# YyzHarry/imbalanced-regression

Hardware: NVIDIA H100
Metric: images/sec (higher is better)
Workload: dtype bf16

## Files before the change

imbalanced-regression_b200/csrc/conv_igemm.cu:

```cuda
#include <stdlib.h>
#include "common.cuh"
#include "tc.cuh"
#include "conv.cuh"

namespace dirb200 {
using namespace tc;

constexpr int BM = 128;
constexpr int BK = 64;
constexpr int kProducerThreads = 128;
constexpr int kThreads = 384;
constexpr int kMaxTaps = 25;
constexpr int kMaxSmemBytes = 232448;

struct IgemmParams {
  const __nv_bfloat16* src;
  int n, hs, ws, cs;
  int hm, wm;
  int kh, kw, stride, pad;
  int transposed;
  int cls_on, cls_py, cls_px, full_h, full_w;
  int ntaps_c;
  int tap_list[kMaxTaps];
  long long tap_eoff[kMaxTaps];
  unsigned short tap_r[kMaxTaps], tap_s[kMaxTaps];
  FastDiv fd_hw, fd_wm, fd_cpb, fd_kw, fd_ntiles, fd_persplit;
  int cpb;
  long long pixels;
  int num_kblocks;
  int kblocks_per_split;
  int total_chunks;
  int m_tiles, n_tiles;
  int num_tiles;
  int a_mode;
  int i2c_stride, i2c_lo;
  int ldc;
  void* out;
  float* stat_out;
  const float* epi_scale;
  const float* epi_shift;
  const __nv_bfloat16* epi_res;
  int epi_relu;
  const __nv_bfloat16* bst_y;
  const float* bst_scale;
  const float* bst_shift;
};

template <int BN, bool STAGED_EPI>
struct Cfg {
  static constexpr int kABytes = BM * BK * 2;
  static constexpr int kBBytes = BN * BK * 2;
  static constexpr int kStageBytes = kABytes + kBBytes;
  static constexpr int kStages = BN == 128 ? (STAGED_EPI ? 5 : 6) : 8;
  static constexpr int kBarOffset = kStages * kStageBytes;
  static constexpr int kStageRowBytes = BN * 2 + 16;
  static constexpr int kEpiWarpBytes = 16 * kStageRowBytes;
  static constexpr int kEpiOffset = kBarOffset + 256;
  static constexpr int kStatWarpBytes = 2 * BN * 4;
  static constexpr int kStatOffset = kEpiOffset + (STAGED_EPI ? 8 * kEpiWarpBytes : 0);
  static constexpr int kSmemBytes = kStatOffset + (STAGED_EPI ? 8 * kStatWarpBytes : 0) + 1024;
  static_assert(kSmemBytes <= kMaxSmemBytes, "shared memory budget");
};

__device__ __forceinline__ uint32_t pack_pixel(long long p, const IgemmParams& P) {
  if (p >= P.pixels) return 0u;
  uint32_t n, rem, y, x;
  P.fd_hw.divmod(static_cast<uint32_t>(p), n, rem);
  P.fd_wm.divmod(rem, y, x);
  return 0x80000000u | (n << 18) | (y << 9) | x;
}

struct RowPre {
  int nb, yb, xb;
};
__device__ __forceinline__ RowPre row_pre(const IgemmParams& P, uint32_t pk) {
  RowPre rp;
  const int n = (pk >> 18) & 0x1FFF;
  int y = (pk >> 9) & 0x1FF, x = pk & 0x1FF;
  if (P.cls_on) {
    y = 2 * y + P.cls_py;
    x = 2 * x + P.cls_px;
  }
  rp.nb = n * P.hs;
  if (!P.transposed) {
    rp.yb = y * P.stride - P.pad;
    rp.xb = x * P.stride - P.pad;
  } else {
    rp.yb = y + P.pad;
    rp.xb = x + P.pad;
  }
  if (!(pk >> 31)) rp.yb = -(1 << 28);
  return rp;
}

__device__ __forceinline__ const __nv_bfloat16* tap_source(const IgemmParams& P, const RowPre& rp, int r, int s,
                                                           int coff, bool& ok) {
  int hi, wi;
  ok = true;
  if (!P.transposed) {
    hi = rp.yb + r;
    wi = rp.xb + s;
  } else {
    hi = rp.yb - r;
    wi = rp.xb - s;
    if (P.stride == 2) {
      ok = ((hi | wi) & 1) == 0;
      hi >>= 1;
      wi >>= 1;
    }
  }
  ok = ok && static_cast<unsigned>(hi) < static_cast<unsigned>(P.hs) &&
       static_cast<unsigned>(wi) < static_cast<unsigned>(P.ws);
  return ok ? P.src + (static_cast<size_t>(rp.nb + hi) * P.ws + wi) * P.cs + coff : P.src;
}
template <int BN, bool WGRAD, bool STEM, bool ATMA = false, bool AFFINE = false, bool BSTAT = false>
__global__ void __launch_bounds__(kThreads, 1)
igemm_kernel(const __grid_constant__ CUtensorMap tmap_b, const __grid_constant__ CUtensorMap tmap_a,
             const IgemmParams P) {
  using C = Cfg<BN, !WGRAD>;
  static_assert(BN == 64 || BN == 128, "tile width: one m64n64 / m64n128 wgmma per warpgroup and k step");
  static_assert(!ATMA || !STEM, "TMA-fed A operand: not for the stem");
  static_assert(!AFFINE || (!WGRAD && !STEM), "folded-BN epilogue: non-stem fprop GEMMs only");
  static_assert(!BSTAT || (ATMA && !WGRAD && !AFFINE), "BN-backward moments in the epilogue: TMA-fed dgrad GEMMs only");
  extern __shared__ uint8_t smem_raw[];
  const uint32_t smem_base = (smem_u32(smem_raw) + 1023u) & ~1023u;
  uint8_t* const smem_gen = smem_raw + (smem_base - smem_u32(smem_raw));
  const uint32_t bar_base = smem_base + C::kBarOffset;
  auto a_addr = [&](int s) { return smem_base + s * C::kStageBytes; };
  auto b_addr = [&](int s) { return smem_base + s * C::kStageBytes + C::kABytes; };
  constexpr uint32_t nstages = C::kStages;
  auto full_bar = [&](int s) { return bar_base + 8u * s; };
  auto empty_bar = [&](int s) { return bar_base + 8u * (C::kStages + s); };
  const int warp = static_cast<int>(threadIdx.x >> 5), lane = threadIdx.x & 31;

  int tile_first, tile_end, tile_step, fixed_n = 0;
  if constexpr (WGRAD) {
    tile_first = blockIdx.x; tile_end = P.num_tiles; tile_step = gridDim.x;
  } else {
    uint32_t gi, nn;
    P.fd_ntiles.divmod(blockIdx.x, gi, nn);
    fixed_n = static_cast<int>(nn);
    tile_first = static_cast<int>(gi);
    tile_end = P.m_tiles;
    tile_step = static_cast<int>(P.fd_ntiles.div(gridDim.x - 1u - nn)) + 1;
  }
  auto decode_tile = [&](int t, int& split, int& m_tile, int& n_tile, int& kb_begin, int& nk) {
    if constexpr (WGRAD) {
      uint32_t sp, rem, mt, nt;
      P.fd_persplit.divmod(static_cast<uint32_t>(t), sp, rem);
      P.fd_ntiles.divmod(rem, mt, nt);
      split = static_cast<int>(sp);
      m_tile = static_cast<int>(mt);
      n_tile = static_cast<int>(nt);
      kb_begin = split * P.kblocks_per_split;
      const int kb_end = min(P.num_kblocks, kb_begin + P.kblocks_per_split);
      nk = max(0, kb_end - kb_begin);
    } else {
      split = 0;
      m_tile = t;
      n_tile = fixed_n;
      kb_begin = 0;
      nk = P.num_kblocks;
    }
  };

  if (threadIdx.x == 0) {
    for (int s = 0; s < C::kStages; ++s) {
      mbar_init(full_bar(s), ATMA ? 1 : kProducerThreads + 1);
      mbar_init(empty_bar(s), 8);
    }
    fence_barrier_init();
  }
  __syncthreads();

  if (warp < 4) {
    if constexpr (!ATMA) {
      const int j = lane & 7;
      const int q = lane >> 3;
      uint32_t rs = 0, rph = 0;
      for (int t = tile_first; t < tile_end; t += tile_step) {
        int split, m_tile, n_tile, kb_begin, nk;
        decode_tile(t, split, m_tile, n_tile, kb_begin, nk);
        const int n0 = n_tile * BN;
        long long off8[8];
        uint32_t mask8[8];
        int chunk_r = 0, chunk_s = 0, chunk_c0 = 0;
        bool chunk_ok = true;
        uint32_t tile_off = 0;
        if constexpr (!WGRAD) {
          const RowPre rp = row_pre(P, pack_pixel(static_cast<long long>(m_tile) * BM + warp * 32 + lane, P));
          const bool rvalid = rp.yb > -(1 << 27);
          int oy = rp.yb, ox = rp.xb;
          if (P.transposed && P.stride == 2) { oy >>= 1; ox >>= 1; }
          const long long my_off = (static_cast<long long>(rp.nb + oy) * P.ws + ox) * P.cs;
          uint32_t vy = 0, vx = 0;
          if (rvalid) {
            const int nky = P.kh, nkx = STEM ? 4 : P.kw;
            for (int r = 0; r < nky; ++r) {
              int h = P.transposed ? rp.yb - r : rp.yb + r;
              bool ok = true;
              if (P.transposed && P.stride == 2) { ok = (h & 1) == 0; h >>= 1; }
              vy |= (ok && static_cast<unsigned>(h) < static_cast<unsigned>(P.hs) ? 1u : 0u) << r;
            }
            for (int c = 0; c < nkx; ++c) {
              int w = P.transposed ? rp.xb - c : rp.xb + c;
              bool ok = true;
              if (P.transposed && P.stride == 2) { ok = (w & 1) == 0; w >>= 1; }
              vx |= (ok && static_cast<unsigned>(w) < static_cast<unsigned>(P.ws) ? 1u : 0u) << c;
            }
          }
          uint32_t my_mask;
          if constexpr (STEM) {
            my_mask = vy | (vx << 8);
          } else {
            my_mask = 0;
            for (int r = 0; r < P.kh; ++r)
              if ((vy >> r) & 1u) my_mask |= vx << (r * P.kw);
          }
#pragma unroll
          for (int i = 0; i < 8; ++i) {
            const int row = 4 * i + q;
            const long long o = __shfl_sync(0xffffffffu, my_off, row);
            const uint32_t m = __shfl_sync(0xffffffffu, my_mask, row);
            if constexpr (STEM) {
              off8[i] = o + (j >> 1) * P.cs + (j & 1) * 8;
              mask8[i] = ((m >> (8 + (j >> 1))) & 1u) ? (m & 0xFu) : 0u;
            } else {
              off8[i] = o + j * 8;
              mask8[i] = m;
            }
          }
          tile_off = warp * 32 * 128;
        } else {
          const int chunk = warp >> 1;
          const int gchunk = m_tile * 2 + chunk;
          chunk_ok = gchunk < P.total_chunks;
          if constexpr (STEM) {
            chunk_r = gchunk;
          } else {
            uint32_t tap, cb, cr, csx;
            P.fd_cpb.divmod(static_cast<uint32_t>(gchunk), tap, cb);
            P.fd_kw.divmod(tap, cr, csx);
            chunk_c0 = static_cast<int>(cb) * 64;
            chunk_r = static_cast<int>(cr);
            chunk_s = static_cast<int>(csx);
          }
          tile_off = chunk * 8192 + (warp & 1) * 32 * 128;
        }
        int tc = 0, cb = 0;
        long long stem_toff = 0;
        for (int it = 0; it < nk; ++it) {
          const int s = static_cast<int>(rs);
          mbar_wait(empty_bar(s), rph ^ 1u);
          if (++rs == nstages) { rs = 0; rph ^= 1u; }
          const int kb = kb_begin + it;
          const uint32_t dst_base = a_addr(s) + tile_off;
          int kcoord = kb;
          if constexpr (!WGRAD) {
            int tp;
            long long toff;
            if constexpr (STEM) {
              tp = kb;
              toff = stem_toff;
              stem_toff += static_cast<long long>(P.ws) * P.cs;
            } else {
              tp = P.tap_list[tc];
              toff = P.tap_eoff[tc] + cb * 64;
              kcoord = tp * P.cpb + cb;
              if (++cb == P.cpb) { cb = 0; ++tc; }
            }
#pragma unroll
            for (int i = 0; i < 8; ++i) {
              const int row = 4 * i + q;
              const bool ok = (mask8[i] >> tp) & 1u;
              const __nv_bfloat16* src = ok ? P.src + (off8[i] + toff) : P.src;
              cp_async16(dst_base + row * 128 + ((j ^ (row & 7)) << 4), src, ok ? 16u : 0u);
            }
          } else {
            const uint32_t mypk = chunk_ok ? pack_pixel(static_cast<long long>(kb) * 64 + (warp & 1) * 32 + lane, P) : 0u;
            const RowPre rp = row_pre(P, mypk);
            bool myok;
            const __nv_bfloat16* myptr = tap_source(P, rp, chunk_r, STEM ? 0 : chunk_s, STEM ? 0 : chunk_c0, myok);
            const unsigned long long myaddr = reinterpret_cast<unsigned long long>(myptr);
            uint32_t okbits;
            if constexpr (STEM) {
              okbits = 0;
              const bool rowok = (mypk >> 31) && static_cast<unsigned>(rp.yb + chunk_r) < static_cast<unsigned>(P.hs);
              for (int sp = 0; sp < 4; ++sp)
                okbits |= (rowok && static_cast<unsigned>(rp.xb + sp) < static_cast<unsigned>(P.ws) ? 1u : 0u) << sp;
            } else {
              okbits = myok ? 1u : 0u;
            }
            unsigned long long rowaddr = myaddr;
            if constexpr (STEM)
              rowaddr = reinterpret_cast<unsigned long long>(
                  P.src + ((static_cast<long long>(rp.nb + rp.yb + chunk_r) * P.ws + rp.xb) * P.cs));
#pragma unroll
            for (int i = 0; i < 8; ++i) {
              const int row = 4 * i + q;
              const unsigned long long a = __shfl_sync(0xffffffffu, rowaddr, row);
              const uint32_t okb = __shfl_sync(0xffffffffu, okbits, row);
              const bool ok = STEM ? ((okb >> (j >> 1)) & 1u) : (okb & 1u);
              const __nv_bfloat16* src = reinterpret_cast<const __nv_bfloat16*>(a) + j * 8;
              cp_async16(dst_base + row * 128 + ((j ^ (row & 7)) << 4), ok ? src : P.src, ok ? 16u : 0u);
            }
          }
          if (warp == 0) {
            if (elect_one()) {
              mbar_arrive_expect_tx(full_bar(s), C::kBBytes);
              if constexpr (!WGRAD) {
                tma_load_2d(b_addr(s), &tmap_b, full_bar(s), kcoord * BK, n0);
              } else {
#pragma unroll
                for (int i = 0; i < BN / 64; ++i)
                  tma_load_2d(b_addr(s) + i * 8192, &tmap_b, full_bar(s), n0 + 64 * i, kb * 64);
              }
            }
            __syncwarp();
          }
          cp_async_mbar_arrive_noinc(full_bar(s));
        }
      }
    } else if (warp == 0) {
      uint32_t rs = 0, rph = 0;
      for (int t = tile_first; t < tile_end; t += tile_step) {
        int split, m_tile, n_tile, kb_begin, nk;
        decode_tile(t, split, m_tile, n_tile, kb_begin, nk);
        const int n0 = n_tile * BN;
        int tile_w0 = 0, tile_h0 = 0, tile_n0 = 0;
        if constexpr (!WGRAD) {
          if (P.a_mode == 2) {
            uint32_t tn, rem, y0, x0;
            P.fd_hw.divmod(static_cast<uint32_t>(m_tile) * BM, tn, rem);
            P.fd_wm.divmod(rem, y0, x0);
            tile_n0 = static_cast<int>(tn);
            tile_w0 = static_cast<int>(x0) * P.i2c_stride + P.i2c_lo;
            tile_h0 = static_cast<int>(y0) * P.i2c_stride + P.i2c_lo;
          }
        }
        int tc = 0, cb = 0;
        for (int it = 0; it < nk; ++it) {
          const int s = static_cast<int>(rs);
          mbar_wait(empty_bar(s), rph ^ 1u);
          if (++rs == nstages) { rs = 0; rph ^= 1u; }
          const int kb = kb_begin + it;
          if (elect_one()) {
            if constexpr (!WGRAD) {
              mbar_arrive_expect_tx(full_bar(s), C::kBBytes + C::kABytes);
              if (P.a_mode == 1)
                tma_load_2d(a_addr(s), &tmap_a, full_bar(s), kb * BK, m_tile * BM);
              else
                tma_load_im2col_4d(a_addr(s), &tmap_a, full_bar(s), cb * BK, tile_w0, tile_h0, tile_n0,
                                   P.tap_s[tc], P.tap_r[tc]);
              tma_load_2d(b_addr(s), &tmap_b, full_bar(s), (P.tap_list[tc] * P.cpb + cb) * BK, n0);
            } else {
              const int nchunks = min(2, P.total_chunks - 2 * m_tile);
              mbar_arrive_expect_tx(full_bar(s), C::kBBytes + nchunks * 8192);
              if (P.a_mode == 1) {
                for (int i = 0; i < nchunks; ++i)
                  tma_load_2d(a_addr(s) + i * 8192, &tmap_a, full_bar(s), (2 * m_tile + i) * 64, kb * 64);
              } else {
                uint32_t n0i, rem, y0, x0;
                P.fd_hw.divmod(static_cast<uint32_t>(kb) * 64u, n0i, rem);
                P.fd_wm.divmod(rem, y0, x0);
                for (int i = 0; i < nchunks; ++i) {
                  uint32_t tap, cbk, r, sx;
                  P.fd_cpb.divmod(static_cast<uint32_t>(2 * m_tile + i), tap, cbk);
                  P.fd_kw.divmod(tap, r, sx);
                  tma_load_im2col_4d(a_addr(s) + i * 8192, &tmap_a, full_bar(s), static_cast<int>(cbk) * 64,
                                     static_cast<int>(x0) * P.i2c_stride + P.i2c_lo,
                                     static_cast<int>(y0) * P.i2c_stride + P.i2c_lo, static_cast<int>(n0i),
                                     static_cast<uint16_t>(sx), static_cast<uint16_t>(r));
                }
              }
#pragma unroll
              for (int i = 0; i < BN / 64; ++i)
                tma_load_2d(b_addr(s) + i * 8192, &tmap_b, full_bar(s), n0 + 64 * i, kb * 64);
            }
          }
          if constexpr (!WGRAD) {
            if (++cb == P.cpb) { cb = 0; ++tc; }
          }
          __syncwarp();
        }
      }
    }
    return;
  }

  const int g = (warp >> 2) - 1;
  const int wq = warp & 3;
  const int ew = g * 4 + wq;
  const int fr = lane >> 2, fc = 2 * (lane & 3);
  float* const stat_sm = reinterpret_cast<float*>(smem_gen + C::kStatOffset) + ew * (2 * BN);
  if constexpr (!WGRAD) {
    if (P.stat_out != nullptr)
      for (int i = lane; i < 2 * BN; i += 32) stat_sm[i] = 0.f;
  }
  constexpr uint32_t kLbo = WGRAD ? 8192u : 16u;
  constexpr uint32_t kadv = WGRAD ? (2048u >> 4) : (32u >> 4);
  constexpr int kT = WGRAD ? 1 : 0;
  float acc[BN / 2];
  uint32_t rs = 0, rph = 0;
  for (int t = tile_first; t < tile_end; t += tile_step) {
    int split, m_tile, n_tile, kb_begin, nk;
    decode_tile(t, split, m_tile, n_tile, kb_begin, nk);
    int prev = 0;
    for (int it = 0; it < nk; ++it) {
      const int s = static_cast<int>(rs);
      mbar_wait(full_bar(s), rph);
      if (++rs == nstages) { rs = 0; rph ^= 1u; }
      if constexpr (!ATMA) fence_proxy_async();
      const uint64_t adesc = make_smem_desc(a_addr(s) + g * 8192, kLbo, 1024u);
      const uint64_t bdesc = make_smem_desc(b_addr(s), kLbo, 1024u);
      wgmma_fence_operands(acc);
      wgmma_fence();
#pragma unroll
      for (int k = 0; k < BK / 16; ++k)
        wgmma_bf16<BN, kT, kT>(acc, adesc + static_cast<uint64_t>(k * kadv), bdesc + static_cast<uint64_t>(k * kadv),
                               (it > 0 || k > 0) ? 1u : 0u);
      wgmma_commit();
      wgmma_fence_operands(acc);
      if (it > 0) {
        wgmma_wait<1>();
        if (lane == 0) mbar_arrive(empty_bar(prev));
      }
      prev = s;
    }
    wgmma_wait<0>();
    wgmma_fence_operands(acc);
    if (nk > 0 && lane == 0) mbar_arrive(empty_bar(prev));
    const int n0 = n_tile * BN;

    if constexpr (!WGRAD) {
      const uint32_t stage_base = smem_base + C::kEpiOffset + ew * C::kEpiWarpBytes;
      const bool relu_now = AFFINE && P.epi_relu && P.epi_res == nullptr;
#pragma unroll
      for (int j = 0; j < BN / 8; ++j) {
        const int col = 8 * j + fc;
        float v0 = acc[4 * j], v1 = acc[4 * j + 1], v2 = acc[4 * j + 2], v3 = acc[4 * j + 3];
        if constexpr (AFFINE) {
          const float2 a = __ldg(reinterpret_cast<const float2*>(P.epi_scale + n0 + col));
          const float2 b = __ldg(reinterpret_cast<const float2*>(P.epi_shift + n0 + col));
          v0 = fmaf(v0, a.x, b.x); v1 = fmaf(v1, a.y, b.y); v2 = fmaf(v2, a.x, b.x); v3 = fmaf(v3, a.y, b.y);
          if (relu_now) { v0 = fmaxf(v0, 0.f); v1 = fmaxf(v1, 0.f); v2 = fmaxf(v2, 0.f); v3 = fmaxf(v3, 0.f); }
        }
        __nv_bfloat162 h0 = __floats2bfloat162_rn(v0, v1), h1 = __floats2bfloat162_rn(v2, v3);
        asm volatile("st.shared.b32 [%0], %1;" ::"r"(stage_base + fr * C::kStageRowBytes + col * 2),
                     "r"(*reinterpret_cast<uint32_t*>(&h0)) : "memory");
        asm volatile("st.shared.b32 [%0], %1;" ::"r"(stage_base + (fr + 8) * C::kStageRowBytes + col * 2),
                     "r"(*reinterpret_cast<uint32_t*>(&h1)) : "memory");
      }
      __syncwarp();
      constexpr int kLanesPerRow = BN * 2 / 16;
      constexpr int kRowsPerIter = 32 / kLanesPerRow;
      constexpr int kIters = 16 / kRowsPerIter;
      const int sub = lane / kLanesPerRow, col16 = lane % kLanesPerRow;
      const long long p0 = static_cast<long long>(m_tile) * BM + g * 64 + wq * 16;
      __nv_bfloat16* out_cols = reinterpret_cast<__nv_bfloat16*>(P.out) + n0 + col16 * 8;
#pragma unroll
      for (int i = 0; i < kIters; ++i) {
        const int rl = i * kRowsPerIter + sub;
        const long long p = p0 + rl;
        int orow = (p < P.pixels && nk > 0) ? static_cast<int>(p) : -1;
        if (orow >= 0 && P.cls_on) {
          const uint32_t pk = pack_pixel(p, P);
          const int n = (pk >> 18) & 0x1FFF, yy = (pk >> 9) & 0x1FF, xx = pk & 0x1FF;
          orow = (n * P.full_h + 2 * yy + P.cls_py) * P.full_w + 2 * xx + P.cls_px;
        }
        if (orow >= 0) {
          uint4 val;
          asm volatile("ld.shared.v4.b32 {%0, %1, %2, %3}, [%4];"
                       : "=r"(val.x), "=r"(val.y), "=r"(val.z), "=r"(val.w)
                       : "r"(stage_base + rl * C::kStageRowBytes + col16 * 16));
          if constexpr (AFFINE) {
            if (P.epi_res != nullptr) {
              const uint4 rv = *reinterpret_cast<const uint4*>(P.epi_res + n0 + col16 * 8 + static_cast<long long>(orow) * P.ldc);
              uint32_t o[4] = {val.x, val.y, val.z, val.w};
              const uint32_t rr[4] = {rv.x, rv.y, rv.z, rv.w};
#pragma unroll
              for (int e = 0; e < 4; ++e) {
                float lo = __uint_as_float(o[e] << 16) + __uint_as_float(rr[e] << 16);
                float hi = __uint_as_float(o[e] & 0xffff0000u) + __uint_as_float(rr[e] & 0xffff0000u);
                if (P.epi_relu) { lo = fmaxf(lo, 0.f); hi = fmaxf(hi, 0.f); }
                __nv_bfloat162 h = __floats2bfloat162_rn(lo, hi);
                o[e] = *reinterpret_cast<uint32_t*>(&h);
              }
              val = make_uint4(o[0], o[1], o[2], o[3]);
            }
          }
          *reinterpret_cast<uint4*>(out_cols + static_cast<long long>(orow) * P.ldc) = val;
        }
      }
      if (BSTAT || P.stat_out != nullptr) {
#pragma unroll
        for (int h = 0; h < BN / 64; ++h) {
          const int col = 2 * (lane + 32 * h);
          float s0 = 0.f, s1 = 0.f, q0 = 0.f, q1 = 0.f;
          float2 bsc = make_float2(0.f, 0.f), bsh = bsc;
          if constexpr (BSTAT) {
            bsc = __ldg(reinterpret_cast<const float2*>(P.bst_scale + n0 + col));
            bsh = __ldg(reinterpret_cast<const float2*>(P.bst_shift + n0 + col));
          }
#pragma unroll
          for (int r = 0; r < 16; ++r) {
            uint32_t w;
            asm volatile("ld.shared.b32 %0, [%1];" : "=r"(w) : "r"(stage_base + r * C::kStageRowBytes + col * 2));
            float g0 = __uint_as_float(w << 16), g1 = __uint_as_float(w & 0xffff0000u);
            if constexpr (BSTAT) {
              const long long p = p0 + r;
              const uint32_t yw = p < P.pixels ? __ldg(reinterpret_cast<const unsigned int*>(P.bst_y + p * P.ldc + n0 + col)) : 0u;
              const float y0 = __uint_as_float(yw << 16), y1 = __uint_as_float(yw & 0xffff0000u);
              if (!(fmaf(y0, bsc.x, bsh.x) > 0.f)) g0 = 0.f;
              if (!(fmaf(y1, bsc.y, bsh.y) > 0.f)) g1 = 0.f;
              s0 += g0; s1 += g1;
              q0 = fmaf(g0, y0, q0); q1 = fmaf(g1, y1, q1);
            } else {
              s0 += g0; s1 += g1;
              q0 = fmaf(g0, g0, q0); q1 = fmaf(g1, g1, q1);
            }
          }
          stat_sm[col] += s0;
          stat_sm[col + 1] += s1;
          stat_sm[BN + col] += q0;
          stat_sm[BN + col + 1] += q1;
        }
      }
      __syncwarp();
    } else {
      const int ktot = P.total_chunks * 64;
      const int krow = m_tile * BM + g * 64 + wq * 16 + fr;
      float* out = reinterpret_cast<float*>(P.out) + (static_cast<size_t>(split) * P.ldc + n0) * ktot;
#pragma unroll
      for (int j = 0; j < BN / 8; ++j) {
        const size_t c0 = static_cast<size_t>(8 * j + fc) * ktot;
#pragma unroll
        for (int e = 0; e < 2; ++e) {
          if (krow < ktot) out[c0 + e * ktot + krow] = nk > 0 ? acc[4 * j + e] : 0.f;
          if (krow + 8 < ktot) out[c0 + e * ktot + krow + 8] = nk > 0 ? acc[4 * j + 2 + e] : 0.f;
        }
      }
    }
  }
  if constexpr (!WGRAD) {
    if (P.stat_out != nullptr) {
      asm volatile("bar.sync 1, 256;" ::: "memory");
      const float* all = reinterpret_cast<const float*>(smem_gen + C::kStatOffset);
      float* dst = P.stat_out + static_cast<size_t>(blockIdx.x) * 2 * P.ldc + fixed_n * BN;
      for (int o = static_cast<int>(threadIdx.x) - kProducerThreads; o < 2 * BN; o += kThreads - kProducerThreads) {
        const int k = o / BN, col = o - k * BN;
        const float v = ((all[o] + all[2 * BN + o]) + (all[4 * BN + o] + all[6 * BN + o])) +
                        ((all[8 * BN + o] + all[10 * BN + o]) + (all[12 * BN + o] + all[14 * BN + o]));
        dst[static_cast<size_t>(k) * P.ldc + col] = v;
      }
    }
  }
}

typedef CUresult (*EncodeTiledFn)(CUtensorMap*, CUtensorMapDataType, cuuint32_t, void*, const cuuint64_t*,
                                  const cuuint64_t*, const cuuint32_t*, const cuuint32_t*, CUtensorMapInterleave,
                                  CUtensorMapSwizzle, CUtensorMapL2promotion, CUtensorMapFloatOOBfill);

static EncodeTiledFn encode_fn() {
  static EncodeTiledFn fn = nullptr;
  if (!fn) {
    void* p = nullptr;
    cudaDriverEntryPointQueryResult q;
    if (cudaGetDriverEntryPoint("cuTensorMapEncodeTiled", &p, cudaEnableDefault, &q) == cudaSuccess &&
        q == cudaDriverEntryPointSuccess)
      fn = reinterpret_cast<EncodeTiledFn>(p);
  }
  return fn;
}

int make_tmap_bf16_2d(CUtensorMap* tm, const void* ptr, uint64_t inner, uint64_t outer, uint64_t row_stride_bytes,
                      uint32_t box_outer) {
  EncodeTiledFn fn = encode_fn();
  if (!fn) {
    set_error("cuTensorMapEncodeTiled entry point not available");
    return DIRB200_ERR_CUDA;
  }
  cuuint64_t dims[2] = {inner, outer};
  cuuint64_t strides[1] = {row_stride_bytes};
  cuuint32_t box[2] = {64, box_outer};
  cuuint32_t estr[2] = {1, 1};
  CUresult r = fn(tm, CU_TENSOR_MAP_DATA_TYPE_BFLOAT16, 2, const_cast<void*>(ptr), dims, strides, box, estr,
                  CU_TENSOR_MAP_INTERLEAVE_NONE, CU_TENSOR_MAP_SWIZZLE_128B, CU_TENSOR_MAP_L2_PROMOTION_L2_256B,
                  CU_TENSOR_MAP_FLOAT_OOB_FILL_NONE);
  if (r != CUDA_SUCCESS) {
    set_error("cuTensorMapEncodeTiled failed (%d) inner=%llu outer=%llu stride=%llu", (int)r,
              (unsigned long long)inner, (unsigned long long)outer, (unsigned long long)row_stride_bytes);
    return DIRB200_ERR_CUDA;
  }
  return DIRB200_OK;
}

typedef CUresult (*EncodeIm2colFn)(CUtensorMap*, CUtensorMapDataType, cuuint32_t, void*, const cuuint64_t*,
                                   const cuuint64_t*, const int*, const int*, cuuint32_t, cuuint32_t, const cuuint32_t*,
                                   CUtensorMapInterleave, CUtensorMapSwizzle, CUtensorMapL2promotion,
                                   CUtensorMapFloatOOBfill);
int make_tmap_im2col_bf16(CUtensorMap* tm, const void* ptr, int c, int w, int h, int n, int lower_w, int lower_h,
                          int upper_w, int upper_h, int trav, int pixels_per_col) {
  static EncodeIm2colFn fn = nullptr;
  if (!fn) {
    void* p = nullptr;
    cudaDriverEntryPointQueryResult q;
    if (cudaGetDriverEntryPoint("cuTensorMapEncodeIm2col", &p, cudaEnableDefault, &q) == cudaSuccess &&
        q == cudaDriverEntryPointSuccess)
      fn = reinterpret_cast<EncodeIm2colFn>(p);
  }
  if (!fn) {
    set_error("cuTensorMapEncodeIm2col entry point not available");
    return DIRB200_ERR_CUDA;
  }
  cuuint64_t dims[4] = {(cuuint64_t)c, (cuuint64_t)w, (cuuint64_t)h, (cuuint64_t)n};
  cuuint64_t strides[3] = {(cuuint64_t)c * 2, (cuuint64_t)w * c * 2, (cuuint64_t)h * w * c * 2};
  int lower[2] = {lower_w, lower_h}, upper[2] = {upper_w, upper_h};
  cuuint32_t estr[4] = {1, (cuuint32_t)trav, (cuuint32_t)trav, 1};
  CUresult r = fn(tm, CU_TENSOR_MAP_DATA_TYPE_BFLOAT16, 4, const_cast<void*>(ptr), dims, strides, lower, upper, 64,
                  (cuuint32_t)pixels_per_col, estr, CU_TENSOR_MAP_INTERLEAVE_NONE, CU_TENSOR_MAP_SWIZZLE_128B,
                  CU_TENSOR_MAP_L2_PROMOTION_L2_256B, CU_TENSOR_MAP_FLOAT_OOB_FILL_NONE);
  if (r != CUDA_SUCCESS) {
    set_error("cuTensorMapEncodeIm2col failed (%d) c=%d w=%d h=%d n=%d lower=%d,%d upper=%d,%d stride=%d", (int)r, c, w, h,
              n, lower_w, lower_h, upper_w, upper_h, trav);
    return DIRB200_ERR_CUDA;
  }
  int drv = 0;
  if (cudaDriverGetVersion(&drv) == cudaSuccess && drv <= 13010 && (size_t)c * w * h * n * 2 < 131072)
    reinterpret_cast<uint64_t*>(tm)[1] &= ~(1ull << 21);
  return DIRB200_OK;
}
static thread_local StatLayout t_last_layout{};

static IgemmParams finish_params(const IgemmParams& P) {
  IgemmParams Q = P;
  Q.fd_hw = make_fastdiv(static_cast<uint32_t>(Q.hm * Q.wm));
  Q.fd_wm = make_fastdiv(static_cast<uint32_t>(Q.wm));
  Q.fd_cpb = make_fastdiv(static_cast<uint32_t>(Q.cpb > 0 ? Q.cpb : 1));
  Q.fd_kw = make_fastdiv(static_cast<uint32_t>(Q.kw > 0 ? Q.kw : 1));
  Q.fd_ntiles = make_fastdiv(static_cast<uint32_t>(Q.n_tiles > 0 ? Q.n_tiles : 1));
  Q.fd_persplit = make_fastdiv(static_cast<uint32_t>(Q.m_tiles * Q.n_tiles > 0 ? Q.m_tiles * Q.n_tiles : 1));
  const int nt = Q.ntaps_c < kMaxTaps ? Q.ntaps_c : kMaxTaps;
  for (int i = 0; i < kMaxTaps; ++i) {
    Q.tap_eoff[i] = 0;
    Q.tap_r[i] = Q.tap_s[i] = 0;
  }
  for (int i = 0; i < nt && Q.kw > 0; ++i) {
    const int tp = Q.tap_list[i];
    int r = tp / Q.kw, sx = tp - r * Q.kw;
    if (Q.transposed && Q.cls_on) {
      Q.tap_r[i] = static_cast<unsigned short>((Q.cls_py + Q.pad - r) / 2 - Q.i2c_lo);
      Q.tap_s[i] = static_cast<unsigned short>((Q.cls_px + Q.pad - sx) / 2 - Q.i2c_lo);
      r >>= 1; sx >>= 1;
      Q.tap_eoff[i] = -static_cast<long long>(r * Q.ws + sx) * Q.cs;
    } else if (Q.transposed) {
      Q.tap_r[i] = static_cast<unsigned short>(Q.kh - 1 - r);
      Q.tap_s[i] = static_cast<unsigned short>(Q.kw - 1 - sx);
      if (Q.stride == 2) { r >>= 1; sx >>= 1; }
      Q.tap_eoff[i] = -static_cast<long long>(r * Q.ws + sx) * Q.cs;
    } else {
      Q.tap_r[i] = static_cast<unsigned short>(r);
      Q.tap_s[i] = static_cast<unsigned short>(sx);
      Q.tap_eoff[i] = static_cast<long long>(r * Q.ws + sx) * Q.cs;
    }
  }
  return Q;
}

template <int BN, bool WGRAD, bool STEM, bool ATMA = false, bool AFFINE = false, bool BSTAT = false>
static int launch_igemm_impl(const CUtensorMap& tm, const CUtensorMap& tma, const IgemmParams& Qin, cudaStream_t st) {
  using C = Cfg<BN, !WGRAD>;
  const IgemmParams Q = finish_params(Qin);
  static bool configured = false;
  if (!configured) {
    DIRB_CUDA(cudaFuncSetAttribute(igemm_kernel<BN, WGRAD, STEM, ATMA, AFFINE, BSTAT>,
                                   cudaFuncAttributeMaxDynamicSharedMemorySize, C::kSmemBytes));
    configured = true;
  }
  int grid = Q.num_tiles < num_sms() ? Q.num_tiles : num_sms();
  if (!WGRAD && grid < Q.n_tiles) grid = Q.n_tiles;
  t_last_layout = StatLayout{grid, Q.n_tiles, BN, 1};
  igemm_kernel<BN, WGRAD, STEM, ATMA, AFFINE, BSTAT><<<grid, kThreads, C::kSmemBytes, st>>>(tm, tma, Q);
  DIRB_LAUNCHED();
  return DIRB200_OK;
}

template <int BN, bool WGRAD, bool STEM>
static int launch_igemm(const CUtensorMap& tm, const IgemmParams& P, int m_tiles, int splits, cudaStream_t st,
                        const CUtensorMap* tma = nullptr) {
  IgemmParams Q = P;
  Q.m_tiles = m_tiles;
  Q.num_tiles = m_tiles * P.n_tiles * splits;
  if constexpr (!STEM) {
    if (tma) {
      if constexpr (!WGRAD) {
        if (Q.epi_scale != nullptr) return launch_igemm_impl<BN, false, false, true, true>(tm, *tma, Q, st);
        if (Q.bst_y != nullptr) return launch_igemm_impl<BN, false, false, true, false, true>(tm, *tma, Q, st);
      }
      return launch_igemm_impl<BN, WGRAD, false, true>(tm, *tma, Q, st);
    }
  }
  if constexpr (!WGRAD && !STEM) {
    if (Q.epi_scale != nullptr) return launch_igemm_impl<BN, false, false, false, true>(tm, tm, Q, st);
  }
  if (Q.epi_scale != nullptr || Q.bst_y != nullptr) {
    set_error("conv: the BN-backward moments epilogue needs a TMA-fed A operand; the folded-BN one a non-stem fprop");
// ... 304 lines not shown
```

imbalanced-regression_b200/csrc/tc.cuh:

```cuda
#pragma once
#include <cuda.h>
#include <stdint.h>

namespace dirb200 {
namespace tc {

__device__ __forceinline__ uint32_t smem_u32(const void* p) {
  return static_cast<uint32_t>(__cvta_generic_to_shared(p));
}

__device__ __forceinline__ void mbar_init(uint32_t bar, uint32_t count) {
  asm volatile("mbarrier.init.shared::cta.b64 [%0], %1;" ::"r"(bar), "r"(count) : "memory");
}
__device__ __forceinline__ void fence_barrier_init() {
  asm volatile("fence.mbarrier_init.release.cluster;" ::: "memory");
}
__device__ __forceinline__ void mbar_arrive(uint32_t bar) {
  asm volatile("mbarrier.arrive.shared::cta.b64 _, [%0];" ::"r"(bar) : "memory");
}
__device__ __forceinline__ void mbar_arrive_expect_tx(uint32_t bar, uint32_t bytes) {
  asm volatile("mbarrier.arrive.expect_tx.shared::cta.b64 _, [%0], %1;" ::"r"(bar), "r"(bytes) : "memory");
}
__device__ __forceinline__ bool mbar_try_wait(uint32_t bar, uint32_t parity) {
  uint32_t ok;
  asm volatile(
      "{\n"
      ".reg .pred p;\n"
      "mbarrier.try_wait.parity.shared::cta.b64 p, [%1], %2;\n"
      "selp.u32 %0, 1, 0, p;\n"
      "}\n"
      : "=r"(ok)
      : "r"(bar), "r"(parity)
      : "memory");
  return ok != 0;
}
__device__ __forceinline__ void mbar_wait(uint32_t bar, uint32_t parity) {
  if (mbar_try_wait(bar, parity)) return;
  unsigned long long t0;
  asm volatile("mov.u64 %0, %%globaltimer;" : "=l"(t0));
  while (!mbar_try_wait(bar, parity)) {
    unsigned long long t1;
    asm volatile("mov.u64 %0, %%globaltimer;" : "=l"(t1));
    if (t1 - t0 > 4000000000ull) __trap();
  }
}

__device__ __forceinline__ bool elect_one() {
  uint32_t pred;
  asm volatile(
      "{\n"
      ".reg .pred P;\n"
      "elect.sync _|P, 0xffffffff;\n"
      "selp.u32 %0, 1, 0, P;\n"
      "}\n"
      : "=r"(pred));
  return pred != 0;
}

__device__ __forceinline__ void cp_async16(uint32_t dst, const void* src, uint32_t src_bytes) {
  asm volatile("cp.async.cg.shared.global [%0], [%1], 16, %2;" ::"r"(dst), "l"(src), "r"(src_bytes) : "memory");
}
__device__ __forceinline__ void cp_async_mbar_arrive_noinc(uint32_t bar) {
  asm volatile("cp.async.mbarrier.arrive.noinc.shared::cta.b64 [%0];" ::"r"(bar) : "memory");
}
__device__ __forceinline__ void fence_proxy_async() { asm volatile("fence.proxy.async.shared::cta;" ::: "memory"); }

__device__ __forceinline__ void tma_load_2d(uint32_t dst, const CUtensorMap* tmap, uint32_t bar, int c0, int c1) {
  asm volatile(
      "cp.async.bulk.tensor.2d.shared::cluster.global.mbarrier::complete_tx::bytes [%0], [%1, {%3, %4}], [%2];"
      ::"r"(dst), "l"(tmap), "r"(bar), "r"(c0), "r"(c1)
      : "memory");
}

__device__ __forceinline__ void tma_load_im2col_4d(uint32_t dst, const CUtensorMap* tmap, uint32_t bar, int c, int w,
                                                   int h, int n, uint16_t off_w, uint16_t off_h) {
  asm volatile(
      "cp.async.bulk.tensor.4d.shared::cluster.global.im2col.mbarrier::complete_tx::bytes"
      " [%0], [%1, {%3, %4, %5, %6}], [%2], {%7, %8};"
      ::"r"(dst), "l"(tmap), "r"(bar), "r"(c), "r"(w), "r"(h), "r"(n), "h"(off_w), "h"(off_h)
      : "memory");
}

__device__ __forceinline__ void wgmma_fence() { asm volatile("wgmma.fence.sync.aligned;" ::: "memory"); }
__device__ __forceinline__ void wgmma_commit() { asm volatile("wgmma.commit_group.sync.aligned;" ::: "memory"); }
template <int N>
__device__ __forceinline__ void wgmma_wait() {
  asm volatile("wgmma.wait_group.sync.aligned %0;" ::"n"(N) : "memory");
}
template <int R>
__device__ __forceinline__ void wgmma_fence_operands(float (&d)[R]) {
#pragma unroll
  for (int i = 0; i < R; ++i) asm volatile("" : "+f"(d[i])::"memory");
}

#define DIRB_F4(i) "+f"(d[i]), "+f"(d[i + 1]), "+f"(d[i + 2]), "+f"(d[i + 3])
#define DIRB_F16(i) DIRB_F4(i), DIRB_F4(i + 4), DIRB_F4(i + 8), DIRB_F4(i + 12)
#define DIRB_R8(a, b, c, e, f, g, h, k) "%" #a ", %" #b ", %" #c ", %" #e ", %" #f ", %" #g ", %" #h ", %" #k ", "
template <int TA, int TB>
__device__ __forceinline__ void wgmma_m64n64(float (&d)[32], uint64_t adesc, uint64_t bdesc, uint32_t accumulate) {
  asm volatile(
      "{\n.reg .pred p;\nsetp.ne.b32 p, %34, 0;\n"
      "wgmma.mma_async.sync.aligned.m64n64k16.f32.bf16.bf16 {"
      DIRB_R8(0, 1, 2, 3, 4, 5, 6, 7) DIRB_R8(8, 9, 10, 11, 12, 13, 14, 15) DIRB_R8(16, 17, 18, 19, 20, 21, 22, 23)
      "%24, %25, %26, %27, %28, %29, %30, %31}, %32, %33, p, 1, 1, %35, %36;\n}\n"
      : DIRB_F16(0), DIRB_F16(16)
      : "l"(adesc), "l"(bdesc), "r"(accumulate), "n"(TA), "n"(TB));
}
template <int TA, int TB>
__device__ __forceinline__ void wgmma_m64n128(float (&d)[64], uint64_t adesc, uint64_t bdesc, uint32_t accumulate) {
  asm volatile(
      "{\n.reg .pred p;\nsetp.ne.b32 p, %66, 0;\n"
      "wgmma.mma_async.sync.aligned.m64n128k16.f32.bf16.bf16 {"
      DIRB_R8(0, 1, 2, 3, 4, 5, 6, 7) DIRB_R8(8, 9, 10, 11, 12, 13, 14, 15) DIRB_R8(16, 17, 18, 19, 20, 21, 22, 23)
      DIRB_R8(24, 25, 26, 27, 28, 29, 30, 31) DIRB_R8(32, 33, 34, 35, 36, 37, 38, 39) DIRB_R8(40, 41, 42, 43, 44, 45, 46, 47)
      DIRB_R8(48, 49, 50, 51, 52, 53, 54, 55)
      "%56, %57, %58, %59, %60, %61, %62, %63}, %64, %65, p, 1, 1, %67, %68;\n}\n"
      : DIRB_F16(0), DIRB_F16(16), DIRB_F16(32), DIRB_F16(48)
      : "l"(adesc), "l"(bdesc), "r"(accumulate), "n"(TA), "n"(TB));
}
#undef DIRB_R8
#undef DIRB_F16
#undef DIRB_F4
template <int BN, int TA, int TB>
__device__ __forceinline__ void wgmma_bf16(float (&d)[BN / 2], uint64_t adesc, uint64_t bdesc, uint32_t accumulate) {
  if constexpr (BN == 128) wgmma_m64n128<TA, TB>(d, adesc, bdesc, accumulate);
  else wgmma_m64n64<TA, TB>(d, adesc, bdesc, accumulate);
}

__device__ __forceinline__ uint64_t make_smem_desc(uint32_t saddr, uint32_t lbo_bytes, uint32_t sbo_bytes) {
  uint64_t d = 0;
  d |= static_cast<uint64_t>((saddr & 0x3FFFFu) >> 4);
  d |= static_cast<uint64_t>((lbo_bytes >> 4) & 0x3FFFu) << 16;
  d |= static_cast<uint64_t>((sbo_bytes >> 4) & 0x3FFFu) << 32;
  d |= static_cast<uint64_t>(1) << 62;
  return d;
}

}
}
```

Before: 6177.

## Ping-pong consumer warpgroups over whole tiles with register reallocation

```diff
diff --git a/imbalanced-regression_b200/csrc/conv_igemm.cu b/imbalanced-regression_b200/csrc/conv_igemm.cu
--- a/imbalanced-regression_b200/csrc/conv_igemm.cu
+++ b/imbalanced-regression_b200/csrc/conv_igemm.cu
@@ -10,6 +10,7 @@
 constexpr int BK = 64;
 constexpr int kProducerThreads = 128;
 constexpr int kThreads = 384;
+constexpr uint32_t kBarStatFlush = 1, kBarMmaTurn = 2, kBarStatTurn = 4;
 constexpr int kMaxTaps = 25;
 constexpr int kMaxSmemBytes = 232448;
 
@@ -133,17 +134,19 @@
   auto empty_bar = [&](int s) { return bar_base + 8u * (C::kStages + s); };
   const int warp = static_cast<int>(threadIdx.x >> 5), lane = threadIdx.x & 31;
 
-  int tile_first, tile_end, tile_step, fixed_n = 0;
-  if constexpr (WGRAD) {
-    tile_first = blockIdx.x; tile_end = P.num_tiles; tile_step = gridDim.x;
-  } else {
-    uint32_t gi, nn;
-    P.fd_ntiles.divmod(blockIdx.x, gi, nn);
-    fixed_n = static_cast<int>(nn);
-    tile_first = static_cast<int>(gi);
-    tile_end = P.m_tiles;
-    tile_step = static_cast<int>(P.fd_ntiles.div(gridDim.x - 1u - nn)) + 1;
-  }
+  int tile_first = 0, tile_end = 0, tile_step = 1, fixed_n = 0;
+  auto init_walk = [&]() {
+    if constexpr (WGRAD) {
+      tile_first = blockIdx.x; tile_end = P.num_tiles; tile_step = gridDim.x;
+    } else {
+      uint32_t gi, nn;
+      P.fd_ntiles.divmod(blockIdx.x, gi, nn);
+      fixed_n = static_cast<int>(nn);
+      tile_first = static_cast<int>(gi);
+      tile_end = P.m_tiles;
+      tile_step = static_cast<int>(P.fd_ntiles.div(gridDim.x - 1u - nn)) + 1;
+    }
+  };
   auto decode_tile = [&](int t, int& split, int& m_tile, int& n_tile, int& kb_begin, int& nk) {
     if constexpr (WGRAD) {
       uint32_t sp, rem, mt, nt;
@@ -167,13 +170,25 @@
   if (threadIdx.x == 0) {
     for (int s = 0; s < C::kStages; ++s) {
       mbar_init(full_bar(s), ATMA ? 1 : kProducerThreads + 1);
-      mbar_init(empty_bar(s), 8);
+      mbar_init(empty_bar(s), 4);
     }
     fence_barrier_init();
   }
+  if constexpr (!WGRAD) {
+    if (P.stat_out != nullptr) {
+      float* const all = reinterpret_cast<float*>(smem_gen + C::kStatOffset);
+      for (int i = threadIdx.x; i < 8 * 2 * BN; i += kThreads) all[i] = 0.f;
+    }
+  }
   __syncthreads();
 
+  constexpr uint32_t kProducerRegs = ATMA ? 24 : 72;
+  constexpr uint32_t kConsumerRegs = ATMA ? 240 : 216;
+  static_assert(128 * kProducerRegs + 256 * kConsumerRegs <= 65536, "register file");
+
   if (warp < 4) {
+    setmaxnreg_dec<kProducerRegs>();
+    init_walk();
     if constexpr (!ATMA) {
       const int j = lane & 7;
       const int q = lane >> 3;
@@ -387,171 +402,231 @@
     }
     return;
   }
+  setmaxnreg_inc<kConsumerRegs>();
+  init_walk();
 
   const int g = (warp >> 2) - 1;
   const int wq = warp & 3;
   const int ew = g * 4 + wq;
   const int fr = lane >> 2, fc = 2 * (lane & 3);
-  float* const stat_sm = reinterpret_cast<float*>(smem_gen + C::kStatOffset) + ew * (2 * BN);
-  if constexpr (!WGRAD) {
-    if (P.stat_out != nullptr)
-      for (int i = lane; i < 2 * BN; i += 32) stat_sm[i] = 0.f;
-  }
+  float* const stat_all = reinterpret_cast<float*>(smem_gen + C::kStatOffset);
+  auto stat_slot = [&](int h) { return stat_all + (h * 4 + wq) * (2 * BN); };
   constexpr uint32_t kLbo = WGRAD ? 8192u : 16u;
   constexpr uint32_t kadv = WGRAD ? (2048u >> 4) : (32u >> 4);
   constexpr int kT = WGRAD ? 1 : 0;
-  float acc[BN / 2];
+  float acc[2][BN / 2];
   uint32_t rs = 0, rph = 0;
-  for (int t = tile_first; t < tile_end; t += tile_step) {
+  auto skip_kblocks = [&](int n) {
+    const uint32_t pos = rs + static_cast<uint32_t>(n);
+    rph ^= (pos / nstages) & 1u;
+    rs = pos % nstages;
+  };
+  auto tile_kblocks = [&](int t) {
     int split, m_tile, n_tile, kb_begin, nk;
     decode_tile(t, split, m_tile, n_tile, kb_begin, nk);
+    return nk;
+  };
+  int t = tile_first;
+  if (g == 1 && t < tile_end) {
+    skip_kblocks(tile_kblocks(t));
+    t += tile_step;
+  }
+  for (; t < tile_end; t += 2 * tile_step) {
+    int split, m_tile, n_tile, kb_begin, nk;
+    decode_tile(t, split, m_tile, n_tile, kb_begin, nk);
+    const bool has_prev = t != tile_first;
+    const bool has_next = t + tile_step < tile_end;
+    if (has_prev) named_bar_sync(kBarMmaTurn + g, 256);
     int prev = 0;
     for (int it = 0; it < nk; ++it) {
       const int s = static_cast<int>(rs);
       mbar_wait(full_bar(s), rph);
       if (++rs == nstages) { rs = 0; rph ^= 1u; }
       if constexpr (!ATMA) fence_proxy_async();
-      const uint64_t adesc = make_smem_desc(a_addr(s) + g * 8192, kLbo, 1024u);
+      const uint64_t adesc = make_smem_desc(a_addr(s), kLbo, 1024u);
       const uint64_t bdesc = make_smem_desc(b_addr(s), kLbo, 1024u);
-      wgmma_fence_operands(acc);
+      wgmma_fence_operands(acc[0]);
+      wgmma_fence_operands(acc[1]);
       wgmma_fence();
 #pragma unroll
-      for (int k = 0; k < BK / 16; ++k)
-        wgmma_bf16<BN, kT, kT>(acc, adesc + static_cast<uint64_t>(k * kadv), bdesc + static_cast<uint64_t>(k * kadv),
-                               (it > 0 || k > 0) ? 1u : 0u);
+      for (int k = 0; k < BK / 16; ++k) {
+#pragma unroll
+        for (int h = 0; h < 2; ++h)
+          wgmma_bf16<BN, kT, kT>(acc[h], adesc + static_cast<uint64_t>(h * (8192 >> 4) + k * kadv),
+                                 bdesc + static_cast<uint64_t>(k * kadv), (it > 0 || k > 0) ? 1u : 0u);
+      }
       wgmma_commit();
-      wgmma_fence_operands(acc);
+      wgmma_fence_operands(acc[0]);
+      wgmma_fence_operands(acc[1]);
       if (it > 0) {
         wgmma_wait<1>();
         if (lane == 0) mbar_arrive(empty_bar(prev));
       }
       prev = s;
     }
+    if (has_next) {
+      named_bar_arrive(kBarMmaTurn + (g ^ 1), 256);
+      skip_kblocks(tile_kblocks(t + tile_step));
+    }
     wgmma_wait<0>();
-    wgmma_fence_operands(acc);
+    wgmma_fence_operands(acc[0]);
+    wgmma_fence_operands(acc[1]);
     if (nk > 0 && lane == 0) mbar_arrive(empty_bar(prev));
     const int n0 = n_tile * BN;
 
     if constexpr (!WGRAD) {
       const uint32_t stage_base = smem_base + C::kEpiOffset + ew * C::kEpiWarpBytes;
       const bool relu_now = AFFINE && P.epi_relu && P.epi_res == nullptr;
-#pragma unroll
-      for (int j = 0; j < BN / 8; ++j) {
-        const int col = 8 * j + fc;
-        float v0 = acc[4 * j], v1 = acc[4 * j + 1], v2 = acc[4 * j + 2], v3 = acc[4 * j + 3];
-        if constexpr (AFFINE) {
-          const float2 a = __ldg(reinterpret_cast<const float2*>(P.epi_scale + n0 + col));
-          const float2 b = __ldg(reinterpret_cast<const float2*>(P.epi_shift + n0 + col));
-          v0 = fmaf(v0, a.x, b.x); v1 = fmaf(v1, a.y, b.y); v2 = fmaf(v2, a.x, b.x); v3 = fmaf(v3, a.y, b.y);
-          if (relu_now) { v0 = fmaxf(v0, 0.f); v1 = fmaxf(v1, 0.f); v2 = fmaxf(v2, 0.f); v3 = fmaxf(v3, 0.f); }
-        }
-        __nv_bfloat162 h0 = __floats2bfloat162_rn(v0, v1), h1 = __floats2bfloat162_rn(v2, v3);
-        asm volatile("st.shared.b32 [%0], %1;" ::"r"(stage_base + fr * C::kStageRowBytes + col * 2),
-                     "r"(*reinterpret_cast<uint32_t*>(&h0)) : "memory");
-        asm volatile("st.shared.b32 [%0], %1;" ::"r"(stage_base + (fr + 8) * C::kStageRowBytes + col * 2),
-                     "r"(*reinterpret_cast<uint32_t*>(&h1)) : "memory");
-      }
-      __syncwarp();
+      const bool stats = BSTAT || P.stat_out != nullptr;
       constexpr int kLanesPerRow = BN * 2 / 16;
       constexpr int kRowsPerIter = 32 / kLanesPerRow;
       constexpr int kIters = 16 / kRowsPerIter;
       const int sub = lane / kLanesPerRow, col16 = lane % kLanesPerRow;
-      const long long p0 = static_cast<long long>(m_tile) * BM + g * 64 + wq * 16;
       __nv_bfloat16* out_cols = reinterpret_cast<__nv_bfloat16*>(P.out) + n0 + col16 * 8;
-#pragma unroll
-      for (int i = 0; i < kIters; ++i) {
-        const int rl = i * kRowsPerIter + sub;
-        const long long p = p0 + rl;
-        int orow = (p < P.pixels && nk > 0) ? static_cast<int>(p) : -1;
-        if (orow >= 0 && P.cls_on) {
-          const uint32_t pk = pack_pixel(p, P);
-          const int n = (pk >> 18) & 0x1FFF, yy = (pk >> 9) & 0x1FF, xx = pk & 0x1FF;
-          orow = (n * P.full_h + 2 * yy + P.cls_py) * P.full_w + 2 * xx + P.cls_px;
-        }
-        if (orow >= 0) {
-          uint4 val;
-          asm volatile("ld.shared.v4.b32 {%0, %1, %2, %3}, [%4];"
-                       : "=r"(val.x), "=r"(val.y), "=r"(val.z), "=r"(val.w)
-                       : "r"(stage_base + rl * C::kStageRowBytes + col16 * 16));
+      uint32_t packed[2][BN / 4];
+#pragma unroll
+      for (int j = 0; j < BN / 8; ++j) {
+        float2 a = make_float2(0.f, 0.f), b = a;
+        if constexpr (AFFINE) {
+          a = __ldg(reinterpret_cast<const float2*>(P.epi_scale + n0 + 8 * j + fc));
+          b = __ldg(reinterpret_cast<const float2*>(P.epi_shift + n0 + 8 * j + fc));
+        }
+#pragma unroll
+        for (int hf = 0; hf < 2; ++hf) {
+          float v0 = acc[hf][4 * j], v1 = acc[hf][4 * j + 1], v2 = acc[hf][4 * j + 2], v3 = acc[hf][4 * j + 3];
           if constexpr (AFFINE) {
-            if (P.epi_res != nullptr) {
-              const uint4 rv = *reinterpret_cast<const uint4*>(P.epi_res + n0 + col16 * 8 + static_cast<long long>(orow) * P.ldc);
-              uint32_t o[4] = {val.x, val.y, val.z, val.w};
-              const uint32_t rr[4] = {rv.x, rv.y, rv.z, rv.w};
-#pragma unroll
-              for (int e = 0; e < 4; ++e) {
-                float lo = __uint_as_float(o[e] << 16) + __uint_as_float(rr[e] << 16);
-                float hi = __uint_as_float(o[e] & 0xffff0000u) + __uint_as_float(rr[e] & 0xffff0000u);
-                if (P.epi_relu) { lo = fmaxf(lo, 0.f); hi = fmaxf(hi, 0.f); }
-                __nv_bfloat162 h = __floats2bfloat162_rn(lo, hi);
-                o[e] = *reinterpret_cast<uint32_t*>(&h);
+            v0 = fmaf(v0, a.x, b.x); v1 = fmaf(v1, a.y, b.y); v2 = fmaf(v2, a.x, b.x); v3 = fmaf(v3, a.y, b.y);
+            if (relu_now) { v0 = fmaxf(v0, 0.f); v1 = fmaxf(v1, 0.f); v2 = fmaxf(v2, 0.f); v3 = fmaxf(v3, 0.f); }
+          }
+          __nv_bfloat162 h0 = __floats2bfloat162_rn(v0, v1), h1 = __floats2bfloat162_rn(v2, v3);
+          packed[hf][2 * j] = *reinterpret_cast<uint32_t*>(&h0);
+          packed[hf][2 * j + 1] = *reinterpret_cast<uint32_t*>(&h1);
+        }
+      }
+      float part[2][BN / 64][4];
+#pragma unroll
+      for (int hf = 0; hf < 2; ++hf) {
+#pragma unroll
+        for (int j = 0; j < BN / 8; ++j) {
+          const int col = 8 * j + fc;
+          asm volatile("st.shared.b32 [%0], %1;" ::"r"(stage_base + fr * C::kStageRowBytes + col * 2),
+                       "r"(packed[hf][2 * j]) : "memory");
+          asm volatile("st.shared.b32 [%0], %1;" ::"r"(stage_base + (fr + 8) * C::kStageRowBytes + col * 2),
+                       "r"(packed[hf][2 * j + 1]) : "memory");
+        }
+        __syncwarp();
+        const long long p0 = static_cast<long long>(m_tile) * BM + hf * 64 + wq * 16;
+#pragma unroll
+        for (int i = 0; i < kIters; ++i) {
+          const int rl = i * kRowsPerIter + sub;
+          const long long p = p0 + rl;
+          int orow = (p < P.pixels && nk > 0) ? static_cast<int>(p) : -1;
+          if (orow >= 0 && P.cls_on) {
+            const uint32_t pk = pack_pixel(p, P);
+            const int n = (pk >> 18) & 0x1FFF, yy = (pk >> 9) & 0x1FF, xx = pk & 0x1FF;
+            orow = (n * P.full_h + 2 * yy + P.cls_py) * P.full_w + 2 * xx + P.cls_px;
+          }
+          if (orow >= 0) {
+            uint4 val;
+            asm volatile("ld.shared.v4.b32 {%0, %1, %2, %3}, [%4];"
+                         : "=r"(val.x), "=r"(val.y), "=r"(val.z), "=r"(val.w)
+                         : "r"(stage_base + rl * C::kStageRowBytes + col16 * 16));
+            if constexpr (AFFINE) {
+              if (P.epi_res != nullptr) {
+                const uint4 rv = *reinterpret_cast<const uint4*>(P.epi_res + n0 + col16 * 8 + static_cast<long long>(orow) * P.ldc);
+                uint32_t o[4] = {val.x, val.y, val.z, val.w};
+                const uint32_t rr[4] = {rv.x, rv.y, rv.z, rv.w};
+#pragma unroll
+                for (int e = 0; e < 4; ++e) {
+                  float lo = __uint_as_float(o[e] << 16) + __uint_as_float(rr[e] << 16);
+                  float hi = __uint_as_float(o[e] & 0xffff0000u) + __uint_as_float(rr[e] & 0xffff0000u);
+                  if (P.epi_relu) { lo = fmaxf(lo, 0.f); hi = fmaxf(hi, 0.f); }
+                  __nv_bfloat162 h = __floats2bfloat162_rn(lo, hi);
+                  o[e] = *reinterpret_cast<uint32_t*>(&h);
+                }
+                val = make_uint4(o[0], o[1], o[2], o[3]);
               }
-              val = make_uint4(o[0], o[1], o[2], o[3]);
-            }
-          }
-          *reinterpret_cast<uint4*>(out_cols + static_cast<long long>(orow) * P.ldc) = val;
-        }
+            }
+            *reinterpret_cast<uint4*>(out_cols + static_cast<long long>(orow) * P.ldc) = val;
+          }
+        }
+        if (stats) {
+#pragma unroll
+          for (int h = 0; h < BN / 64; ++h) {
+            const int col = 2 * (lane + 32 * h);
+            float s0 = 0.f, s1 = 0.f, q0 = 0.f, q1 = 0.f;
+            float2 bsc = make_float2(0.f, 0.f), bsh = bsc;
+            if constexpr (BSTAT) {
+              bsc = __ldg(reinterpret_cast<const float2*>(P.bst_scale + n0 + col));
+              bsh = __ldg(reinterpret_cast<const float2*>(P.bst_shift + n0 + col));
+            }
+#pragma unroll
+            for (int r = 0; r < 16; ++r) {
+              uint32_t w;
+              asm volatile("ld.shared.b32 %0, [%1];" : "=r"(w) : "r"(stage_base + r * C::kStageRowBytes + col * 2));
+              float g0 = __uint_as_float(w << 16), g1 = __uint_as_float(w & 0xffff0000u);
+              if constexpr (BSTAT) {
+                const long long p = p0 + r;
+                uint32_t yw = 0u;
+                if (p < P.pixels)
+                  asm volatile("ld.global.nc.b32 %0, [%1];" : "=r"(yw) : "l"(P.bst_y + p * P.ldc + n0 + col));
+                const float y0 = __uint_as_float(yw << 16), y1 = __uint_as_float(yw & 0xffff0000u);
+                if (!(fmaf(y0, bsc.x, bsh.x) > 0.f)) g0 = 0.f;
+                if (!(fmaf(y1, bsc.y, bsh.y) > 0.f)) g1 = 0.f;
+                s0 += g0; s1 += g1;
+                q0 = fmaf(g0, y0, q0); q1 = fmaf(g1, y1, q1);
+              } else {
+                s0 += g0; s1 += g1;
+                q0 = fmaf(g0, g0, q0); q1 = fmaf(g1, g1, q1);
+              }
+            }
+            part[hf][h][0] = s0; part[hf][h][1] = s1; part[hf][h][2] = q0; part[hf][h][3] = q1;
+          }
+        }
+        __syncwarp();
       }
-      if (BSTAT || P.stat_out != nullptr) {
-#pragma unroll
-        for (int h = 0; h < BN / 64; ++h) {
-          const int col = 2 * (lane + 32 * h);
-          float s0 = 0.f, s1 = 0.f, q0 = 0.f, q1 = 0.f;
-          float2 bsc = make_float2(0.f, 0.f), bsh = bsc;
-          if constexpr (BSTAT) {
-            bsc = __ldg(reinterpret_cast<const float2*>(P.bst_scale + n0 + col));
-            bsh = __ldg(reinterpret_cast<const float2*>(P.bst_shift + n0 + col));
-          }
-#pragma unroll
-          for (int r = 0; r < 16; ++r) {
-            uint32_t w;
-            asm volatile("ld.shared.b32 %0, [%1];" : "=r"(w) : "r"(stage_base + r * C::kStageRowBytes + col * 2));
-            float g0 = __uint_as_float(w << 16), g1 = __uint_as_float(w & 0xffff0000u);
-            if constexpr (BSTAT) {
-              const long long p = p0 + r;
-              const uint32_t yw = p < P.pixels ? __ldg(reinterpret_cast<const unsigned int*>(P.bst_y + p * P.ldc + n0 + col)) : 0u;
-              const float y0 = __uint_as_float(yw << 16), y1 = __uint_as_float(yw & 0xffff0000u);
-              if (!(fmaf(y0, bsc.x, bsh.x) > 0.f)) g0 = 0.f;
-              if (!(fmaf(y1, bsc.y, bsh.y) > 0.f)) g1 = 0.f;
-              s0 += g0; s1 += g1;
-              q0 = fmaf(g0, y0, q0); q1 = fmaf(g1, y1, q1);
-            } else {
-              s0 += g0; s1 += g1;
-              q0 = fmaf(g0, g0, q0); q1 = fmaf(g1, g1, q1);
-            }
-          }
-          stat_sm[col] += s0;
-          stat_sm[col + 1] += s1;
-          stat_sm[BN + col] += q0;
-          stat_sm[BN + col + 1] += q1;
+      if (stats) {
+        if (has_prev) named_bar_sync(kBarStatTurn + g, 256);
+#pragma unroll
+        for (int hf = 0; hf < 2; ++hf) {
+          float* const slot = stat_slot(hf);
+#pragma unroll
+          for (int h = 0; h < BN / 64; ++h) {
+            const int col = 2 * (lane + 32 * h);
+            slot[col] += part[hf][h][0];
+            slot[col + 1] += part[hf][h][1];
+            slot[BN + col] += part[hf][h][2];
+            slot[BN + col + 1] += part[hf][h][3];
+          }
+        }
+        if (has_next) {
+          named_bar_arrive(kBarStatTurn + (g ^ 1), 256);
+        } else {
+          named_bar_sync(kBarStatFlush, 128);
+          float* dst = P.stat_out + static_cast<size_t>(blockIdx.x) * 2 * P.ldc + fixed_n * BN;
+          for (int o = wq * 32 + lane; o < 2 * BN; o += 128) {
+            const int k = o / BN, col = o - k * BN;
+            const float v = ((stat_all[o] + stat_all[2 * BN + o]) + (stat_all[4 * BN + o] + stat_all[6 * BN + o])) +
+                            ((stat_all[8 * BN + o] + stat_all[10 * BN + o]) + (stat_all[12 * BN + o] + stat_all[14 * BN + o]));
+            dst[static_cast<size_t>(k) * P.ldc + col] = v;
+          }
         }
       }
-      __syncwarp();
     } else {
       const int ktot = P.total_chunks * 64;
-      const int krow = m_tile * BM + g * 64 + wq * 16 + fr;
       float* out = reinterpret_cast<float*>(P.out) + (static_cast<size_t>(split) * P.ldc + n0) * ktot;
 #pragma unroll
-      for (int j = 0; j < BN / 8; ++j) {
-        const size_t c0 = static_cast<size_t>(8 * j + fc) * ktot;
-#pragma unroll
-        for (int e = 0; e < 2; ++e) {
-          if (krow < ktot) out[c0 + e * ktot + krow] = nk > 0 ? acc[4 * j + e] : 0.f;
-          if (krow + 8 < ktot) out[c0 + e * ktot + krow + 8] = nk > 0 ? acc[4 * j + 2 + e] : 0.f;
-        }
-      }
-    }
-  }
-  if constexpr (!WGRAD) {
-    if (P.stat_out != nullptr) {
-      asm volatile("bar.sync 1, 256;" ::: "memory");
-      const float* all = reinterpret_cast<const float*>(smem_gen + C::kStatOffset);
-      float* dst = P.stat_out + static_cast<size_t>(blockIdx.x) * 2 * P.ldc + fixed_n * BN;
-      for (int o = static_cast<int>(threadIdx.x) - kProducerThreads; o < 2 * BN; o += kThreads - kProducerThreads) {
-        const int k = o / BN, col = o - k * BN;
-        const float v = ((all[o] + all[2 * BN + o]) + (all[4 * BN + o] + all[6 * BN + o])) +
-                        ((all[8 * BN + o] + all[10 * BN + o]) + (all[12 * BN + o] + all[14 * BN + o]));
-        dst[static_cast<size_t>(k) * P.ldc + col] = v;
+      for (int hf = 0; hf < 2; ++hf) {
+        const int krow = m_tile * BM + hf * 64 + wq * 16 + fr;
+#pragma unroll
+        for (int j = 0; j < BN / 8; ++j) {
+          const size_t c0 = static_cast<size_t>(8 * j + fc) * ktot;
+#pragma unroll
+          for (int e = 0; e < 2; ++e) {
+            if (krow < ktot) out[c0 + e * ktot + krow] = nk > 0 ? acc[hf][4 * j + e] : 0.f;
+            if (krow + 8 < ktot) out[c0 + e * ktot + krow + 8] = nk > 0 ? acc[hf][4 * j + 2 + e] : 0.f;
+          }
+        }
       }
     }
   }
diff --git a/imbalanced-regression_b200/csrc/tc.cuh b/imbalanced-regression_b200/csrc/tc.cuh
--- a/imbalanced-regression_b200/csrc/tc.cuh
+++ b/imbalanced-regression_b200/csrc/tc.cuh
@@ -55,6 +55,22 @@
       "}\n"
       : "=r"(pred));
   return pred != 0;
+}
+
+__device__ __forceinline__ void named_bar_sync(uint32_t id, uint32_t count) {
+  asm volatile("bar.sync %0, %1;" ::"r"(id), "r"(count) : "memory");
+}
+__device__ __forceinline__ void named_bar_arrive(uint32_t id, uint32_t count) {
+  asm volatile("bar.arrive %0, %1;" ::"r"(id), "r"(count) : "memory");
+}
+
+template <uint32_t R>
+__device__ __forceinline__ void setmaxnreg_inc() {
+  asm volatile("setmaxnreg.inc.sync.aligned.u32 %0;" ::"n"(R));
+}
+template <uint32_t R>
+__device__ __forceinline__ void setmaxnreg_dec() {
+  asm volatile("setmaxnreg.dec.sync.aligned.u32 %0;" ::"n"(R));
 }
 
 __device__ __forceinline__ void cp_async16(uint32_t dst, const void* src, uint32_t src_bytes) {
```

Result: no change. 6218, median of 6 (+0.7%).
